# golmschenk/sr-gan

Hardware: AMD Instinct MI355X
Metric: SRGAN train images/sec (G+D step) (higher is better)
Workload: dtype f32; 1 GPU; crowd SRGAN (KnnDenseNetCat D/DNN + DCGenerator) 512x512, batch 16/GPU, dnn_training_step + gan_training_step per step; global_batch=16, image_size=512, schedule=shared-forwards, parallelism=dp1, random_init_weights=True, gradient_penalty=active, launch=eager (Python tape enqueues every kernel), schedule_check=not run: the --full option runs it

## Files before the change

### include/srgan_hip.h

```cpp
#ifndef SRGAN_HIP_H
#define SRGAN_HIP_H

#include <stdint.h>

#ifdef __cplusplus
extern "C" {
#endif

int srgan_version(void);
const char* srgan_build_id(void);
const char* srgan_last_error(void);

#define SRGAN_DTYPE_F32 0x1u
#define SRGAN_DTYPE_BF16 0x2u
#define SRGAN_DTYPE_F16 0x4u
#define SRGAN_FEATURE_FUSED_BNRELU 0x1u
#define SRGAN_FEATURE_SPLITK_WORKSPACE 0x2u
#define SRGAN_FEATURE_LIVE_PROFILE 0x4u
#define SRGAN_FEATURE_BLOCKED16 0x8u
typedef struct srgan_capabilities_t {
  int32_t abi_version;
  int32_t struct_bytes;
  char arch[16];
  uint32_t dtypes;
// ... 46 lines not shown
  float* g_gamma;
  float* g_beta;
} srgan_bn_reduce_job;
int64_t srgan_conv2d_bwd_data_bnrelu_tiles(const srgan_conv_desc* desc);
int srgan_conv2d_bwd_data_bnrelu_partials(const srgan_conv_desc* desc, const float* gy, const float* w, const srgan_bn_relu* bn,
                                          const float* x, float* gx, float* partials, int accumulate, void* stream);
int srgan_bn_partial_reduce_batched(const srgan_bn_reduce_job* jobs_device, int32_t count, int32_t max_channels, int32_t max_tiles,
                                    const float* scratch, void* stream);

int srgan_wgrad_group_plan(const srgan_conv_desc* desc, const srgan_bn_relu* bn, int64_t x_offset, int64_t gy_offset, float* gw,
                           int64_t gw_offset, int32_t group_size, int64_t group_weights, int64_t partial_offset, void* job,
                           int32_t* grid_x, int32_t* grid_y, int32_t* ragged, int64_t* partial_floats);
int srgan_wgrad_group_run(const void* jobs, int32_t count, int32_t kernel_size, int32_t grid_x, int32_t grid_y, int32_t ragged,
                          int32_t fused_bn, const float* x_base, const float* gy_base, float* gw_base, int64_t sum_co_ci_taps,
                          int64_t pixels, int64_t operand_elements, int64_t partial_floats, void* stream);

int srgan_gemm_f32(int32_t M, int32_t N, int32_t K, const float* A, int64_t sai, int64_t sak, const float* B,
                   int64_t sbk, int64_t sbj, float* C, int64_t sci, int64_t scj, const float* bias,
                   int32_t bias_on_columns, int accumulate, int force_kernel, void* stream);
int srgan_gemm(int32_t M, int32_t N, int32_t K, const float* A, int64_t sai, int64_t sak, const float* B,
               int64_t sbk, int64_t sbj, float* C, int64_t sci, int64_t scj, const float* bias,
               int32_t bias_on_columns, int accumulate, int force_kernel, int compute_dtype, void* stream);

int srgan_ew_unary(int op, const float* x, float* y, int64_t n, float p0, float p1, void* stream);
int srgan_ew_binary(int op, const float* a, const float* b, float* y, int64_t n, float p0, void* stream);
int srgan_fill(float* y, int64_t n, float value, void* stream);

int srgan_chan_affine(const float* x, const float* mean, const float* scale_a, const float* scale_b, const float* shift,
                      float* y, int32_t N, int32_t C, int64_t HW, void* stream);

int srgan_chan_affine_act(const float* x, const float* mean, const float* scale_a, const float* scale_b,
                          const float* shift, const float* mask, int relu, float* y, int32_t N, int32_t C, int64_t HW,
                          void* stream);
int srgan_chan_affine_act_strided(const float* x, const float* mean, const float* scale_a, const float* scale_b,
                                  const float* shift, const float* mask, int relu, float* y, int32_t N, int32_t C,
                                  int64_t HW, int64_t x_batch_stride, int64_t mask_batch_stride, int64_t y_batch_stride,
                                  int accumulate, void* stream);
int srgan_bn_conv_tangent_weights(const float* w, const float* q, const float* inv_std, const float* gamma,
                                  float* w_scaled, float* w_grad, float* gamma_grad, int32_t CO, int32_t CI, int32_t taps,
                                  void* stream);

int srgan_bn_conv_tangent_weights_job(const float* w, const float* inv_std, const float* gamma, float* w_grad,
                                      float* gamma_grad, int64_t offset, int32_t CO, int32_t CI, int32_t taps, void* job);
int srgan_bn_conv_tangent_weights_grouped(const void* jobs, int32_t count, int32_t max_inner, int32_t max_co, float* scaled_base,
                                          const float* q_base, void* stream);

int srgan_bn_act_bwd(const float* g, const float* x, const float* mean, const float* inv_std, const float* gamma,
                     const float* beta, int relu, float* gx, float* g_gamma, float* g_beta, int32_t N, int32_t C,
                     int64_t HW, int64_t g_batch_stride, int64_t x_batch_stride, int64_t gx_batch_stride,
                     int accumulate_gx, int unscaled, void* stream);

int srgan_chan_reduce(const float* a, const float* b, const float* mean, const float* scale, float* out, int32_t N,
                      int32_t C, int64_t HW, int accumulate, void* stream);
int srgan_row_max(const float* x, float* out, int32_t B, int32_t F, void* stream);
int srgan_nearest_bin_onehot(const float* y, const float* bins, float* onehot, int32_t B, int32_t K, void* stream);

int srgan_copy_channels(const float* src, int32_t src_channels, int32_t src_first, float* dst, int32_t dst_channels,
                        int32_t dst_first, int32_t count, int32_t N, int64_t HW, int accumulate, void* stream);

int srgan_bn_relu_maxpool_fwd(const float* x, const float* mean, const float* inv_std, const float* gamma, const float* beta,
                              float* y, int32_t* argmax, int32_t N, int32_t C, int32_t H, int32_t W, int32_t k, int32_t s, int32_t p,
                              int32_t OH, int32_t OW, void* stream);
int srgan_bn_relu_maxpool_bwd_supported(int32_t N, int32_t C, int32_t H, int32_t W, int32_t k, int32_t s, int32_t p);
int srgan_bn_relu_maxpool_bwd(const float* gy, const int32_t* argmax, const float* x, const float* mean, const float* inv_std,
                              const float* gamma, const float* beta, float* gx, float* g_gamma, float* g_beta, int32_t N,
                              int32_t C, int32_t H, int32_t W, int32_t k, int32_t s, int32_t p, int32_t OH, int32_t OW,
                              void* stream);
int srgan_bn_relu_avgpool2_supported(int32_t N, int32_t C, int32_t H, int32_t W);
int srgan_bn_relu_avgpool2_fwd(const float* x, const float* mean, const float* inv_std, const float* gamma, const float* beta,
                               float* y, int32_t N, int32_t C, int32_t H, int32_t W, void* stream);
int srgan_bn_relu_avgpool2_bwd(const float* gy, const float* x, const float* mean, const float* inv_std, const float* gamma,
                               const float* beta, float* gx, float* g_gamma, float* g_beta, int32_t N, int32_t C, int32_t H,
                               int32_t W, void* stream);
int srgan_maxpool2d_fwd(const float* x, float* y, int32_t* argmax, int32_t planes, int32_t H, int32_t W, int32_t k,
                        int32_t s, int32_t p, int32_t OH, int32_t OW, void* stream);
int srgan_maxpool2d_bwd(const float* g, const int32_t* argmax, float* gx, int32_t planes, int32_t H, int32_t W, int32_t k,
                        int32_t s, int32_t p, int32_t OH, int32_t OW, void* stream);
int srgan_pool_scatter(const float* g, const int32_t* argmax, float* out, int32_t planes, int64_t in_plane,
                       int64_t out_plane, void* stream);
int srgan_pool_gather(const float* src, const int32_t* argmax, float* out, int32_t planes, int64_t in_plane,
                      int64_t out_plane, void* stream);
int srgan_avgpool2d_fwd(const float* x, float* y, int32_t planes, int32_t H, int32_t W, int32_t k, int32_t s,
                        int32_t OH, int32_t OW, void* stream);
int srgan_avgpool2d_bwd(const float* g, float* gx, int32_t planes, int32_t H, int32_t W, int32_t k, int32_t s,
                        int32_t OH, int32_t OW, void* stream);

int srgan_gp_interpolate(const float* unlabeled, const float* fake, const float* alpha, float* out, int32_t B,
                         int64_t F, void* stream);
int srgan_crowd_map_l1_fwd(const float* maps, const float* target, float* rows, int32_t B, int32_t Cm, int64_t HW,
                           void* stream);
int srgan_crowd_map_l1_bwd(const float* maps, const float* target, const float* g_rows, float* g_maps, int32_t B,
                           int32_t Cm, int64_t HW, void* stream);
int srgan_crowd_extract_patches(const void* const* images_u8, const float* const* labels, const float* const* maps,
                                const int32_t* heights, const int32_t* widths, const int32_t* ys, const int32_t* xs,
                                const int32_t* flips, int32_t B, int32_t P, float* out_images, float* out_labels,
                                float* out_maps, void* stream);

int srgan_crowd_iknn_map(const float* heads_yx, int32_t M, int32_t H, int32_t W, int32_t k, float epsilon, float upper_bound,
                         float* out, void* stream);
int srgan_crowd_density_label(const float* heads, int32_t M, int32_t H, int32_t W, float beta, const float* perspective,
                              int32_t flags, void* workspace, float* out, void* stream);

int srgan_adam_step(float* p, const float* g, float* m, float* v, int64_t n, float lr, float beta1, float beta2,
                    float eps, float weight_decay, int32_t step, void* stream);
int srgan_adam_step_counted(float* p, const float* g, float* m, float* v, int64_t n, float lr, float beta1, float beta2,
                            float eps, float weight_decay, int32_t* state, void* stream);
// ... 62 lines not shown
```

### sr-gan_amd/_lib.py

```python
import ctypes
import os

from ._build import LIBRARY, source_id

c_float_p = ctypes.c_void_p
i32, i64, f32, vp = ctypes.c_int32, ctypes.c_int64, ctypes.c_float, ctypes.c_void_p


class ConvDesc(ctypes.Structure):
    _fields_ = [(name, i32) for name in ('N', 'C', 'H', 'W', 'K', 'R', 'S', 'stride_h', 'stride_w', 'pad_h', 'pad_w',
                                         'OH', 'OW')] + [('x_batch_stride', i64), ('y_batch_stride', i64), ('compute_dtype', i32)]


class BnRelu(ctypes.Structure):
    _fields_ = [(name, vp) for name in ('mean', 'inv_std', 'gamma', 'beta')]


class BnReduceJob(ctypes.Structure):
    _fields_ = [('partial_offset', i64), ('tiles', i32), ('channels', i32), ('inv_std', vp), ('g_gamma', vp), ('g_beta', vp)]


class Capabilities(ctypes.Structure):
    _fields_ = [('abi_version', i32), ('struct_bytes', i32), ('arch', ctypes.c_char * 16), ('dtypes', ctypes.c_uint32),
                ('features', ctypes.c_uint32), ('workspace_bytes', i64), ('max_tensor_elements', i64)]


SIGNATURES = {
    'srgan_version': ([], ctypes.c_int),
    'srgan_build_id': ([], ctypes.c_char_p),
    'srgan_last_error': ([], ctypes.c_char_p),
    'srgan_conv2d_fwd': ([ctypes.POINTER(ConvDesc), vp, vp, vp, vp, ctypes.c_int, vp], ctypes.c_int),
    'srgan_conv2d_bwd_data': ([ctypes.POINTER(ConvDesc), vp, vp, vp, vp, ctypes.c_int, ctypes.c_int, vp],
                              ctypes.c_int),
    'srgan_conv2d_bwd_weight': ([ctypes.POINTER(ConvDesc), vp, vp, vp, ctypes.c_int, ctypes.c_int, vp], ctypes.c_int),
    'srgan_conv2d_bnrelu_supported': ([ctypes.POINTER(ConvDesc), ctypes.c_int], ctypes.c_int),
    'srgan_conv2d_fwd_bnrelu': ([ctypes.POINTER(ConvDesc), vp, ctypes.POINTER(BnRelu), vp, vp, vp, vp], ctypes.c_int),
    'srgan_conv2d_fwd_bnrelu_into_zeros': ([ctypes.POINTER(ConvDesc), vp, ctypes.POINTER(BnRelu), vp, vp, vp, vp],
                                           ctypes.c_int),
    'srgan_conv2d_fwd_bnrelu_splits': ([ctypes.POINTER(ConvDesc)], ctypes.c_int),
    'srgan_bn_conv_tangent_weights': ([vp, vp, vp, vp, vp, vp, vp, i32, i32, i32, vp], ctypes.c_int),
    'srgan_conv2d_bwd_data_bnrelu': ([ctypes.POINTER(ConvDesc), vp, vp, ctypes.POINTER(BnRelu), vp, vp, vp, vp,
                                      ctypes.c_int, vp], ctypes.c_int),
    'srgan_conv2d_bwd_data_bnrelu_tiles': ([ctypes.POINTER(ConvDesc)], ctypes.c_int64),
    'srgan_conv2d_bwd_data_bnrelu_partials': ([ctypes.POINTER(ConvDesc), vp, vp, ctypes.POINTER(BnRelu), vp, vp, vp,
                                               ctypes.c_int, vp], ctypes.c_int),
    'srgan_bn_partial_reduce_batched': ([vp, i32, i32, i32, vp, vp], ctypes.c_int),
    'srgan_conv2d_bwd_weight_bnrelu': ([ctypes.POINTER(ConvDesc), vp, ctypes.POINTER(BnRelu), vp, vp, ctypes.c_int, vp],
                                       ctypes.c_int),
    'srgan_gemm_f32': ([i32, i32, i32, vp, i64, i64, vp, i64, i64, vp, i64, i64, vp, i32, ctypes.c_int, ctypes.c_int,
                        vp], ctypes.c_int),
    'srgan_gemm': ([i32, i32, i32, vp, i64, i64, vp, i64, i64, vp, i64, i64, vp, i32, ctypes.c_int, ctypes.c_int,
                    ctypes.c_int, vp], ctypes.c_int),
    'srgan_ew_unary': ([ctypes.c_int, vp, vp, i64, f32, f32, vp], ctypes.c_int),
    'srgan_ew_binary': ([ctypes.c_int, vp, vp, vp, i64, f32, vp], ctypes.c_int),
    'srgan_fill': ([vp, i64, f32, vp], ctypes.c_int),
    'srgan_chan_affine': ([vp, vp, vp, vp, vp, vp, i32, i32, i64, vp], ctypes.c_int),
    'srgan_chan_affine_act': ([vp, vp, vp, vp, vp, vp, ctypes.c_int, vp, i32, i32, i64, vp], ctypes.c_int),
    'srgan_chan_affine_act_strided': ([vp, vp, vp, vp, vp, vp, ctypes.c_int, vp, i32, i32, i64, i64, i64, i64,
                                       ctypes.c_int, vp], ctypes.c_int),
    'srgan_bn_act_bwd': ([vp, vp, vp, vp, vp, vp, ctypes.c_int, vp, vp, vp, i32, i32, i64, i64, i64, i64, ctypes.c_int,
                          ctypes.c_int, vp],
                         ctypes.c_int),
    'srgan_chan_reduce': ([vp, vp, vp, vp, vp, i32, i32, i64, ctypes.c_int, vp], ctypes.c_int),
    'srgan_row_max': ([vp, vp, i32, i32, vp], ctypes.c_int),
    'srgan_nearest_bin_onehot': ([vp, vp, vp, i32, i32, vp], ctypes.c_int),
    'srgan_copy_channels': ([vp, i32, i32, vp, i32, i32, i32, i32, i64, ctypes.c_int, vp], ctypes.c_int),
    'srgan_bn_relu_maxpool_fwd': ([vp, vp, vp, vp, vp, vp, vp, i32, i32, i32, i32, i32, i32, i32, i32, i32, vp], ctypes.c_int),
    'srgan_bn_relu_maxpool_bwd_supported': ([i32, i32, i32, i32, i32, i32, i32], ctypes.c_int),
    'srgan_bn_relu_maxpool_bwd': ([vp, vp, vp, vp, vp, vp, vp, vp, vp, vp, i32, i32, i32, i32, i32, i32, i32, i32, i32, vp],
                                  ctypes.c_int),
    'srgan_bn_relu_avgpool2_supported': ([i32, i32, i32, i32], ctypes.c_int),
    'srgan_bn_relu_avgpool2_fwd': ([vp, vp, vp, vp, vp, vp, i32, i32, i32, i32, vp], ctypes.c_int),
    'srgan_bn_relu_avgpool2_bwd': ([vp, vp, vp, vp, vp, vp, vp, vp, vp, i32, i32, i32, i32, vp], ctypes.c_int),
    'srgan_maxpool2d_fwd': ([vp, vp, vp, i32, i32, i32, i32, i32, i32, i32, i32, vp], ctypes.c_int),
    'srgan_maxpool2d_bwd': ([vp, vp, vp, i32, i32, i32, i32, i32, i32, i32, i32, vp], ctypes.c_int),
    'srgan_pool_scatter': ([vp, vp, vp, i32, i64, i64, vp], ctypes.c_int),
    'srgan_pool_gather': ([vp, vp, vp, i32, i64, i64, vp], ctypes.c_int),
    'srgan_avgpool2d_fwd': ([vp, vp, i32, i32, i32, i32, i32, i32, i32, vp], ctypes.c_int),
    'srgan_avgpool2d_bwd': ([vp, vp, i32, i32, i32, i32, i32, i32, i32, vp], ctypes.c_int),
    'srgan_gp_interpolate': ([vp, vp, vp, vp, i32, i64, vp], ctypes.c_int),
    'srgan_crowd_map_l1_fwd': ([vp, vp, vp, i32, i32, i64, vp], ctypes.c_int),
    'srgan_crowd_map_l1_bwd': ([vp, vp, vp, vp, i32, i32, i64, vp], ctypes.c_int),
    'srgan_profile_begin': ([], ctypes.c_int),
    'srgan_profile_end': ([ctypes.POINTER(ctypes.c_double), ctypes.POINTER(ctypes.c_double),
                           ctypes.POINTER(ctypes.c_double), ctypes.POINTER(ctypes.c_int64)], ctypes.c_int),
    'srgan_profile_report': ([ctypes.c_char_p, ctypes.c_int64], ctypes.c_int64),
    'srgan_profile_bytes': ([ctypes.POINTER(ctypes.c_double)], ctypes.c_int),
    'srgan_profile_mixed': ([ctypes.POINTER(ctypes.c_double), ctypes.POINTER(ctypes.c_double)], ctypes.c_int),
    'srgan_capabilities': ([ctypes.POINTER(Capabilities), i32], ctypes.c_int),
    'srgan_workspace_bytes': ([], ctypes.c_int64),
    'srgan_set_workspace': ([vp, i64, vp], ctypes.c_int),
    'srgan_split_is_ordered': ([vp], ctypes.c_int),
    'srgan_crowd_density_label': ([vp, i32, i32, i32, f32, vp, i32, vp, vp, vp], ctypes.c_int),
    'srgan_crowd_iknn_map': ([vp, i32, i32, i32, i32, f32, f32, vp, vp], ctypes.c_int),
    'srgan_crowd_extract_patches': ([vp, vp, vp, vp, vp, vp, vp, vp, i32, i32, vp, vp, vp, vp], ctypes.c_int),
    'srgan_bn_conv_tangent_weights_job': ([vp, vp, vp, vp, vp, i64, i32, i32, i32, vp], ctypes.c_int),
    'srgan_bn_conv_tangent_weights_grouped': ([vp, i32, i32, i32, vp, vp, vp], ctypes.c_int),
    'srgan_wgrad_group_plan': ([ctypes.POINTER(ConvDesc), ctypes.POINTER(BnRelu), i64, i64, vp, i64, i32, i64, i64, vp, ctypes.POINTER(i32),
                                ctypes.POINTER(i32), ctypes.POINTER(i32), ctypes.POINTER(i64)], ctypes.c_int),
    'srgan_wgrad_group_run': ([vp, i32, i32, i32, i32, i32, i32, vp, vp, vp, i64, i64, i64, i64, vp], ctypes.c_int),
    'srgan_adam_step': ([vp, vp, vp, vp, i64, f32, f32, f32, f32, f32, i32, vp], ctypes.c_int),
    'srgan_adam_step_counted': ([vp, vp, vp, vp, i64, f32, f32, f32, f32, f32, vp, vp], ctypes.c_int),
    'srgan_pack_bf16': ([vp, vp, i64, vp], ctypes.c_int),
    'srgan_unpack_bf16': ([vp, vp, i64, vp], ctypes.c_int),
    'srgan_h_pack': ([vp, vp, vp, f32, i32, i32, i64, ctypes.c_int, vp], ctypes.c_int),
    'srgan_h_unpack': ([vp, vp, i32, i32, i64, ctypes.c_int, vp], ctypes.c_int),
    'srgan_h_add': ([vp, vp, vp, i64, ctypes.c_int, vp], ctypes.c_int),
    'srgan_h_channel_sums': ([vp, vp, i32, i32, i64, ctypes.c_int, vp], ctypes.c_int),
    'srgan_h_maxpool2': ([vp, vp, vp, i64, i32, i32, ctypes.c_int, ctypes.c_int, vp], ctypes.c_int),
    'srgan_h_maxpool2_bwd': ([vp, vp, vp, i64, i32, i32, ctypes.c_int, f32, ctypes.c_int, vp], ctypes.c_int),
    'srgan_h_conv_weight_slots': ([i32, i32, i32, i32], ctypes.c_int64),
    'srgan_h_pack_conv_weights': ([vp, vp, i32, i32, i32, i32, ctypes.c_int, ctypes.c_int, vp], ctypes.c_int),
    'srgan_h_conv3x3': ([vp, vp, vp, vp, f32, ctypes.c_int, vp, i32, i32, i32, i32, i32, i32, ctypes.c_int, vp], ctypes.c_int),
    'srgan_h_conv3x3_wgrad': ([vp, vp, vp, i32, i32, i32, i32, i32, ctypes.c_int, vp], ctypes.c_int),
    'srgan_h_pack_matrix': ([vp, vp, i64, i64, i64, i64, i64, i64, i32, i32, ctypes.c_int, vp], ctypes.c_int),
# ... 86 lines not shown
```

### sr-gan_amd/crowd/models.py

```python
from collections import OrderedDict

from torch import nn as torch_nn

from .. import functional as F
from .. import nn
from .. import fused
from ..age.models import Generator as _DCGANGenerator, convolution, LEAK
from ..utility import seed_all


FUSED_STEM_POOL = True


class DCGenerator(_DCGANGenerator):

    def __init__(self, z_dim=256, image_size=224, conv_dim=64):
        super().__init__(z_dim=z_dim, image_size=image_size, conv_dim=conv_dim)


class JointDCDiscriminator(nn.Module):

    def __init__(self, image_size=128, conv_dim=64, number_of_outputs=1):
        seed_all(0)
        super().__init__()
        self.number_of_outputs = number_of_outputs
        self.layer1 = convolution(3, conv_dim, 4, bn=False)
        self.layer2 = convolution(conv_dim, conv_dim * 2, 4)
        self.layer3 = convolution(conv_dim * 2, conv_dim * 4, 4)
        self.layer4 = convolution(conv_dim * 4, conv_dim * 8, 4)
        self.count_layer5 = convolution(conv_dim * 8, self.number_of_outputs, int(image_size / 16), 1, 0, False)
        self.density_layer5 = convolution(conv_dim * 8, int(image_size / 4) ** 2, int(image_size / 16), 1, 0, False)
        self.features = None

    def forward(self, x):
        out = x
        for stage in (self.layer1, self.layer2, self.layer3, self.layer4):
            out = F.leaky_relu(stage(out), LEAK)
        self.features = F.flatten2d(out)
        count = self.count_layer5(out)
        count = F.view(count, (-1,) if self.number_of_outputs == 1 else (-1, self.number_of_outputs))
        side = int(x.shape[2] / 4)
        density = F.view(self.density_layer5(out), (-1, side, side))
        return density, count


class _DenseLayer(nn.Sequential):

    def __init__(self, num_input_features, growth_rate, bn_size, drop_rate=0):
        super().__init__()
        self.add_module('norm1', nn.BatchNorm2d(num_input_features))
        self.add_module('relu1', nn.ReLU(inplace=True))
        self.add_module('conv1', nn.Conv2d(num_input_features, bn_size * growth_rate, kernel_size=1, stride=1,
                                           bias=False))
        self.add_module('norm2', nn.BatchNorm2d(bn_size * growth_rate))
        self.add_module('relu2', nn.ReLU(inplace=True))
        self.add_module('conv2', nn.Conv2d(bn_size * growth_rate, growth_rate, kernel_size=3, stride=1, padding=1,
                                           bias=False))
        if drop_rate:
            raise NotImplementedError('drop_rate > 0 is never used on the hot path (crowd/models.py:1063)')
# ... 4 lines not shown


class _DenseBlock(nn.Sequential):
    def __init__(self, num_layers, num_input_features, bn_size, growth_rate, drop_rate=0):
        super().__init__()
        for i in range(num_layers):
            self.add_module('denselayer%d' % (i + 1),
                            _DenseLayer(num_input_features + i * growth_rate, growth_rate, bn_size, drop_rate))

    def forward(self, x):
        if not fused.ENABLED:
            return super().forward(x)
        return fused.dense_block(x, list(self.children()))


class _Transition(nn.Sequential):
    def __init__(self, num_input_features, num_output_features):
        super().__init__()
        self.add_module('norm', nn.BatchNorm2d(num_input_features))
        self.add_module('relu', nn.ReLU(inplace=True))
        self.add_module('conv', nn.Conv2d(num_input_features, num_output_features, kernel_size=1, stride=1,
                                          bias=False))
        self.add_module('pool', nn.AvgPool2d(kernel_size=2, stride=2))

    def forward(self, x):
        if fused.POOL_FIRST:
            pooled = None
            if fused.ENABLED and self.pool.kernel_size == 2 and self.pool.stride == 2:
                inv_std, mean = self.norm._inverse_std()
                pooled = F.bn_relu_avg_pool2d(x, mean, inv_std, nn.P(self.norm.weight), nn.P(self.norm.bias))
            if pooled is None:
                pooled = self.pool(self.norm(x, relu=True))
            return self.conv(pooled)
        y = fused.bn_relu_conv(x, self.norm, self.conv) if fused.ENABLED else None
        if y is None:
            y = self.conv(self.norm(x, relu=True))
        return self.pool(y)


class MapModule(nn.Module):

    def __init__(self, in_features, input_size, label_size, count_outputs=1):
        super().__init__()
        kernel_size = label_size // input_size
        self.map_transposed_conv_layer = nn.ConvTranspose2d(in_channels=in_features, out_channels=1,
                                                            kernel_size=kernel_size, stride=kernel_size)
        self.conv1 = nn.Conv2d(in_channels=1, out_channels=8, kernel_size=2, stride=2)
        self.conv2 = nn.Conv2d(in_channels=8, out_channels=16, kernel_size=2, stride=2)
        self.conv3 = nn.Conv2d(in_channels=16, out_channels=32, kernel_size=2, stride=2)
        self.linear1 = nn.Conv2d(in_channels=32, out_channels=20, kernel_size=label_size // (2 ** 3))
        self.count_layer = nn.Conv2d(in_channels=20, out_channels=count_outputs, kernel_size=1)

    def forward(self, x):
        map_ = F.leaky_relu(self.map_transposed_conv_layer(x))
        out = F.leaky_relu(self.conv1(map_))
        out = F.leaky_relu(self.conv2(out))
        out = F.leaky_relu(self.conv3(out))
        out = F.leaky_relu(self.linear1(out))
        return map_, self.count_layer(out), out


class KnnDenseNetCat(nn.Module):

    COUNT_OUTPUTS = 1

    def __init__(self, growth_rate=32, block_config=(6, 12, 48, 32), num_init_features=64, bn_size=4, drop_rate=0,
                 pretrained=False, label_patch_size=224, image_size=None):
        super().__init__()
        image_size = image_size or label_patch_size
        self.label_patch_size = image_size
        self.dense_blocks = nn.ModuleList()
        self.transition_layers = nn.ModuleList()
        self.conv_layer1 = nn.Sequential(OrderedDict([
            ('conv0', nn.Conv2d(3, num_init_features, kernel_size=7, stride=2, padding=3, bias=False)),
            ('norm0', nn.BatchNorm2d(num_init_features)),
            ('relu0', nn.ReLU(inplace=True)),
            ('pool0', nn.MaxPool2d(kernel_size=3, stride=2, padding=1))]))
        num_features = num_init_features
        widths = []
        for i, num_layers in enumerate(block_config):
            block = _DenseBlock(num_layers=num_layers, num_input_features=num_features, bn_size=bn_size,
                                growth_rate=growth_rate, drop_rate=drop_rate)
            self.dense_blocks.add_module('denseblock%d' % (i + 1), block)
            num_features = num_features + num_layers * growth_rate
            if i != len(block_config) - 1:
                self.transition_layers.add_module('transition%d' % (i + 1),
                                                  _Transition(num_features, num_features // 2))
                num_features = num_features // 2
                widths.append(num_features)
        self.norm5 = nn.BatchNorm2d(num_features)
        for m in self.modules():
            if isinstance(m, torch_nn.Conv2d):
                torch_nn.init.kaiming_normal_(m.weight.data)
            elif isinstance(m, torch_nn.BatchNorm2d):
                m.weight.data.fill_(1)
                m.bias.data.zero_()
            elif isinstance(m, torch_nn.Linear):
                m.bias.data.zero_()
        if pretrained:
            self.load_torchvision_densenet201(pretrained)
        outputs = self.COUNT_OUTPUTS
        self.map_module1 = MapModule(widths[0], image_size // 8, image_size, count_outputs=outputs)
        self.map_module2 = MapModule(widths[1], image_size // 16, image_size, count_outputs=outputs)
        self.map_module3 = MapModule(widths[2], image_size // 32, image_size, count_outputs=outputs)
        self.final_count_feature_layer = nn.Conv2d(in_channels=num_features, out_channels=20, kernel_size=1)
        self.count_layer = nn.Conv2d(in_channels=20, out_channels=outputs, kernel_size=1)
# ... 15 lines not shown
            if match:
                key = match.group(1) + match.group(2)
            key = key.replace('features.denseblock', 'dense_blocks.denseblock')
            key = key.replace('features.transition', 'transition_layers.transition')
            key = key.replace('features.', '') if 'norm5' in key else key.replace('features.', 'conv_layer1.')
            renamed[key] = value
        return renamed

    def load_torchvision_densenet201(self, source=True):
        import os
        if source is True:
            source = os.environ.get(self.TORCHVISION_WEIGHTS_ENV)
            if not source:
                raise RuntimeError('pretrained=True needs the torchvision densenet201 state dict on disk: set '
                                   f'{self.TORCHVISION_WEIGHTS_ENV} to its path (the reference downloads it, '
                                   'crowd/models.py:1110; this build does not touch the network)')
        if isinstance(source, (str, os.PathLike)):
            import torch
            source = torch.load(source, map_location="cpu")
        self.load_state_dict(self.rename_torchvision_keys(source), strict=True)

    def _density(self, batch_size, like):
        cache = self._density_cache
        if cache is None or cache.shape[0] != batch_size or cache.data.device != like.data.device:
            cache = F.full((batch_size, self.label_patch_size, self.label_patch_size), 0.0, like)
            self._density_cache = cache
        return cache

    def forward(self, x):
        count, map_, hidden = self._heads(x)
        batch_size = x.shape[0]
        self.features = F.cat_channels([F.view(t, (batch_size, -1, 1, 1)) for t in hidden])
        return self._density(batch_size, x), F.view(count, (batch_size,)), map_

    def _heads(self, x):
        batch_size = x.shape[0]
        stem = self.conv_layer1
        out, first = None, stem.conv0(x)
        if FUSED_STEM_POOL and isinstance(stem.pool0.kernel_size, int):
            inv_std, mean = stem.norm0._inverse_std()
            out = F.bn_relu_max_pool2d(first, mean, inv_std, nn.parameter_var(stem.norm0.weight),
                                       nn.parameter_var(stem.norm0.bias), stem.pool0.kernel_size, stem.pool0.stride,
                                       stem.pool0.padding)
        if out is None:
            out = stem.pool0(stem.norm0(first, relu=True))
        t1_out = self.transition_layers.transition1(self.dense_blocks.denseblock1(out))
        t2_out = self.transition_layers.transition2(self.dense_blocks.denseblock2(t1_out))
        t3_out = self.transition_layers.transition3(self.dense_blocks.denseblock3(t2_out))
        db4_out = self.dense_blocks.denseblock4(t3_out)
        n5_relu_out = self.norm5(db4_out, relu=True)
        final_pool = F.avg_pool2d(n5_relu_out, kernel_size=self.final_pool_size, stride=1)
        final_count_features = F.leaky_relu(self.final_count_feature_layer(final_pool))
        final_count = self.count_layer(final_count_features)
        map1, count1, h1 = self.map_module1(t1_out)
        map2, count2, h2 = self.map_module2(t2_out)
        map3, count3, h3 = self.map_module3(t3_out)
        count = F.add(F.add(F.add(count1, count2), count3), final_count)
        return count, F.cat_channels([map1, map2, map3]), (h1, h2, h3, final_count_features)


class KnnDenseNetCatDggan(KnnDenseNetCat):
    COUNT_OUTPUTS = 2

    def __init__(self, *args, **kwargs):
        super().__init__(*args, **kwargs)
        self.real_label = None

    def forward(self, x):
        outputs, map_, _ = self._heads(x)
        batch_size = x.shape[0]
        self.real_label = F.view(F.slice_channels(outputs, 1, 2), (batch_size,))
        return self._density(batch_size, x), F.view(F.slice_channels(outputs, 0, 1), (batch_size,)), map_
```

### sr-gan_amd/functional.py

```python
import math
import os

import torch

from . import _lib
from .tape import Var, Node, grad_enabled, no_grad, accumulates_into

U_COPY, U_NEG, U_ABS, U_SIGN, U_SQRT, U_EXP, U_LOG, U_LOG1P, U_SQUARE, U_RECIP, U_TANH, U_RELU, U_STEP, U_AFFINE, \
    U_POW, U_LEAKY, U_SIGMOID, U_SOFTPLUS, U_ONE_MINUS_SQ, U_RSQRT = range(20)
B_ADD, B_SUB, B_MUL, B_DIV, B_DIV_SAFE, B_MAX, B_LEAKY_MASK_MUL, B_AXPY = range(8)

FORCE_KERNEL = 0

COMPUTE_DTYPES = {'f32': 0, 'fp32': 0, 'bf16': 1, 'f16': 2, 'fp16': 2}
COMPUTE_DTYPE = 0


STORAGE_DTYPE = 0
STORAGE_BLOCKED_F32 = 4


class storage_dtype:

    def __init__(self, name):
# ... 173 lines not shown


def sign(x):
    return Var(_unary_raw(U_SIGN, x.data))


def abs_(x):
    return _unary(U_ABS, x, lambda g, needs: (mul(g, sign(x)),), 'abs')


def sqrt(x):
    out = _unary(U_SQRT, x, None, 'sqrt')
    if out.node is not None:
        out.node.backward = lambda g, needs: (div(scale(g, 0.5), out),)
    return out


def exp(x):
    out = _unary(U_EXP, x, None, 'exp')
    if out.node is not None:
        out.node.backward = lambda g, needs: (mul(g, out),)
    return out


def log(x):
    return _unary(U_LOG, x, lambda g, needs: (div(g, x),), 'log')


def log1p(x):
    return _unary(U_LOG1P, x, lambda g, needs: (div(g, add_scalar(x, 1.0)),), 'log1p')


def square(x):
    return _unary(U_SQUARE, x, lambda g, needs: (mul(scale(g, 2.0), x),), 'square')


def one_minus_square(y):
    return _unary(U_ONE_MINUS_SQ, y, lambda g, needs: (scale(mul(g, y), -2.0),), 'one_minus_square')


def tanh(x):
    out = _unary(U_TANH, x, None, 'tanh')
    if out.node is not None:
        out.node.backward = lambda g, needs: (mul(g, one_minus_square(out)),)
    return out


def relu(x):
    return _unary(U_RELU, x, lambda g, needs: (mask_mul(g, x, 0.0),), 'relu')


def leaky_relu(x, negative_slope=0.01):
    return _unary(U_LEAKY, x, lambda g, needs: (mask_mul(g, x, negative_slope),), 'leaky_relu', negative_slope)


def pow_scalar(x, p):
    if p == 2:
        return square(x)
    if p == 1:
        return x
    return _unary(U_POW, x, lambda g, needs: (mul(g, scale(pow_scalar(x, p - 1.0), p)),), 'pow', p)


def sigmoid(x):
    out = _unary(U_SIGMOID, x, None, 'sigmoid')
    if out.node is not None:
        out.node.backward = lambda g, needs: (mul(g, sub(out, square(out))),)
    return out


def softplus(x):
    return _unary(U_SOFTPLUS, x, lambda g, needs: (mul(g, sigmoid(x)),), 'softplus')


def view(x, shape):
    shape = tuple(shape)
    original = x.shape
    return _out(x.data.view(shape), (x,), lambda g, needs: (view(g, original),), 'view')


def flatten2d(x):
    return view(x, (x.shape[0], -1))


def _dims_nchw(shape):
    if len(shape) < 2:
        raise ValueError('need at least [N, C]')
    hw = 1
    for extent in shape[2:]:
        hw *= extent
    return shape[0], shape[1], hw


def chan_affine(x, mean=None, scale_a=None, scale_b=None, shift=None, dims=None, out_shape=None):
    reference = x if x is not None else next(v for v in (scale_a, scale_b, shift) if v is not None)
    if dims is None:
        dims = _dims_nchw(x.shape)
    if out_shape is None:
        out_shape = x.shape
    n, c, hw = dims
    data = _empty(out_shape, reference.data)
    if data.numel() != n * c * hw:
        raise ValueError(f'chan_affine: dims {dims} do not match shape {tuple(out_shape)}')
    for vector in (mean, scale_a, scale_b, shift):
        if vector is not None and vector.numel() != c:
            raise ValueError(f'chan_affine: vector of {vector.numel()} elements for {c} channels')
# ... 101 lines not shown
    return chan_reduce(x, None, dims=(rows, x.numel() // rows, 1))


def row_broadcast(s, shape):
    rows = shape[0]
    count = 1
    for extent in shape[1:]:
        count *= extent
    return chan_affine(None, None, view(s, (rows,)) if s.shape != (rows,) else s, None, None,
                       dims=(1, rows, count), out_shape=tuple(shape))


def col_broadcast(v, rows):
    width = v.numel()
    return chan_affine(None, None, view(v, (width,)) if v.shape != (width,) else v, None, None,
                       dims=(rows, width, 1), out_shape=(rows, width))


def row_norm(x):
    with no_grad():
        out = sqrt(row_dot(x, x))
    if not (grad_enabled() and x.requires_grad):
        return out
    result = Var(out.data, requires_grad=True)
    result.node = Node((x,), lambda g, needs: (row_scale(x, div_safe(g, result)),), 'row_norm')
    return result


def _conv_desc(x_shape, w_shape, stride, padding, y_shape):
    n, c, h, w = x_shape
    k, c2, r, s = w_shape
    if c != c2:
        raise ValueError(f'conv: input has {c} channels, weight expects {c2}')
    return _lib.ConvDesc(n, c, h, w, k, r, s, stride[0], stride[1], padding[0], padding[1], y_shape[2], y_shape[3], 0, 0,
                         COMPUTE_DTYPE)


def _pair(value):
    return (value, value) if isinstance(value, int) else tuple(value)


def conv_output_shape(x_shape, w_shape, stride, padding):
    n, _, h, w = x_shape
    k, _, r, s = w_shape
    return (n, k, (h + 2 * padding[0] - r) // stride[0] + 1, (w + 2 * padding[1] - s) // stride[1] + 1)


def conv2d(x, weight, bias=None, stride=1, padding=0):
    stride, padding = _pair(stride), _pair(padding)
    y_shape = conv_output_shape(x.shape, weight.shape, stride, padding)
    desc = _conv_desc(x.shape, weight.shape, stride, padding, y_shape)
    data = _empty(y_shape, x.data)
    _call('srgan_conv2d_fwd', desc, _ptr(x), _ptr(weight), _ptr(bias), data.data_ptr(), FORCE_KERNEL, _stream())
    x_shape, w_shape = x.shape, weight.shape

    def backward(g, needs):
        gx = conv2d_backward_data(g, weight, x_shape, stride, padding) if needs[0] else None
        gw = gb = None
        if needs[1] and accumulates_into(weight):
            _call('srgan_conv2d_bwd_weight', _conv_desc(x_shape, w_shape, stride, padding, g.shape), _ptr(x), _ptr(g),
                  weight.grad_buffer.data_ptr(), 1, FORCE_KERNEL, _stream())
        elif needs[1]:
            gw = conv2d_backward_weight(x, g, w_shape, stride, padding)
        if needs[2] and accumulates_into(bias):
            _bias_gradient_into(bias.grad_buffer, g)
        elif needs[2]:
            gb = chan_reduce(g)
        return gx, gw, gb
    return _out(data, (x, weight, bias), backward, 'conv2d')


def _bias_gradient_into(buffer, g):
    n, c, hw = _dims_nchw(g.shape)
    _call('srgan_chan_reduce', _ptr(g), None, None, None, buffer.data_ptr(), n, c, hw, 1, _stream())


def conv2d_backward_data(gy, weight, x_shape, stride, padding, bias=None):
    x_shape = tuple(x_shape)
    desc = _conv_desc(x_shape, weight.shape, stride, padding, gy.shape)
    data = _empty(x_shape, gy.data)
    _call('srgan_conv2d_bwd_data', desc, _ptr(gy), _ptr(weight), _ptr(bias), data.data_ptr(), 0, FORCE_KERNEL, _stream())
    w_shape = weight.shape

    def backward(g, needs):
        ggy = conv2d(g, weight, None, stride, padding) if needs[0] else None
        gw = gb = None
        if needs[1] and accumulates_into(weight):
            _call('srgan_conv2d_bwd_weight', _conv_desc(g.shape, w_shape, stride, padding, gy.shape), _ptr(g), _ptr(gy),
                  weight.grad_buffer.data_ptr(), 1, FORCE_KERNEL, _stream())
        elif needs[1]:
            gw = conv2d_backward_weight(g, gy, w_shape, stride, padding)
        if needs[2] and accumulates_into(bias):
            _bias_gradient_into(bias.grad_buffer, g)
        elif needs[2]:
            gb = chan_reduce(g)
        return ggy, gw, gb
    return _out(data, (gy, weight, bias), backward, 'conv2d_backward_data')


def conv2d_backward_weight(x, gy, w_shape, stride, padding):
    w_shape = tuple(w_shape)
    desc = _conv_desc(x.shape, w_shape, stride, padding, gy.shape)
    data = _empty(w_shape, x.data)
    _call('srgan_conv2d_bwd_weight', desc, _ptr(x), _ptr(gy), data.data_ptr(), 0, FORCE_KERNEL, _stream())
    x_shape = x.shape

# ... 294 lines not shown
```

Baseline: 87.68 images/s.

## Fuse the three discriminator map-head forward chains into one grouped HIP kernel

Adds a fused kernel that computes, in a single launch for all three map heads, the leaky ReLU of the transposed-conv output, the three stride-2 2x2 convolutions with leaky ReLU, and the large linear conv as per-block partial sums, followed by a small finish kernel. Each thread walks an 8x8 pixel patch and keeps intermediates in registers and shared memory. The aim is to remove many small eager launches and intermediate round trips through memory. The backward tape is rebuilt from the stored activations. The conv node for the leaky ReLU after a conv is built with the activated data instead of the pre-activation, which relies on the leaky mask sign being the same either way. The path adds register pressure and a serial reduction over blocks.

```diff
diff --git a/include/srgan_hip.h b/include/srgan_hip.h
--- a/include/srgan_hip.h
+++ b/include/srgan_hip.h
@@ -122,6 +122,9 @@
 
 int srgan_chan_reduce(const float* a, const float* b, const float* mean, const float* scale, float* out, int32_t N,
                       int32_t C, int64_t HW, int accumulate, void* stream);
+int64_t srgan_map_head_fwd_workspace(int32_t heads, int32_t B, int32_t S);
+int srgan_map_head_fwd(int32_t heads, const void* const* tensors, float* partial, int32_t B, int32_t S, float slope,
+                       void* stream);
 int srgan_row_max(const float* x, float* out, int32_t B, int32_t F, void* stream);
 int srgan_nearest_bin_onehot(const float* y, const float* bins, float* onehot, int32_t B, int32_t K, void* stream);
 
diff --git a/sr-gan_amd/_lib.py b/sr-gan_amd/_lib.py
--- a/sr-gan_amd/_lib.py
+++ b/sr-gan_amd/_lib.py
@@ -61,6 +61,8 @@
     'srgan_bn_act_bwd': ([vp, vp, vp, vp, vp, vp, ctypes.c_int, vp, vp, vp, i32, i32, i64, i64, i64, i64, ctypes.c_int,
                           ctypes.c_int, vp],
                          ctypes.c_int),
+    'srgan_map_head_fwd_workspace': ([i32, i32, i32], i64),
+    'srgan_map_head_fwd': ([i32, vp, vp, i32, i32, f32, vp], ctypes.c_int),
     'srgan_chan_reduce': ([vp, vp, vp, vp, vp, i32, i32, i64, ctypes.c_int, vp], ctypes.c_int),
     'srgan_row_max': ([vp, vp, i32, i32, vp], ctypes.c_int),
     'srgan_nearest_bin_onehot': ([vp, vp, vp, i32, i32, vp], ctypes.c_int),
diff --git a/sr-gan_amd/crowd/models.py b/sr-gan_amd/crowd/models.py
--- a/sr-gan_amd/crowd/models.py
+++ b/sr-gan_amd/crowd/models.py
@@ -5,6 +5,7 @@
 from .. import functional as F
 from .. import nn
 from .. import fused
+from ..map_head import map_heads
 from ..age.models import Generator as _DCGANGenerator, convolution, LEAK
 from ..utility import seed_all
 
@@ -115,6 +116,9 @@
         self.count_layer = nn.Conv2d(in_channels=20, out_channels=count_outputs, kernel_size=1)
 
     def forward(self, x):
+        return map_heads([self], [x])[0]
+
+    def primitive_forward(self, x):
         map_ = F.leaky_relu(self.map_transposed_conv_layer(x))
         out = F.leaky_relu(self.conv1(map_))
         out = F.leaky_relu(self.conv2(out))
@@ -236,9 +240,8 @@
         final_pool = F.avg_pool2d(n5_relu_out, kernel_size=self.final_pool_size, stride=1)
         final_count_features = F.leaky_relu(self.final_count_feature_layer(final_pool))
         final_count = self.count_layer(final_count_features)
-        map1, count1, h1 = self.map_module1(t1_out)
-        map2, count2, h2 = self.map_module2(t2_out)
-        map3, count3, h3 = self.map_module3(t3_out)
+        (map1, count1, h1), (map2, count2, h2), (map3, count3, h3) = map_heads(
+            [self.map_module1, self.map_module2, self.map_module3], [t1_out, t2_out, t3_out])
         count = F.add(F.add(F.add(count1, count2), count3), final_count)
         return count, F.cat_channels([map1, map2, map3]), (h1, h2, h3, final_count_features)
 
diff --git a/sr-gan_amd/csrc/map_head.hip b/sr-gan_amd/csrc/map_head.hip
--- /dev/null
+++ b/sr-gan_amd/csrc/map_head.hip
@@ -0,0 +1,213 @@
+#include "common.h"
+#include "blocked16.h"
+
+namespace srgan {
+namespace {
+
+constexpr int MH_THREADS = 256;
+constexpr int MH_HIDDEN = 20;
+constexpr int MH_NB = 1;
+constexpr int MH_MAX_HEADS = 3;
+constexpr int W1_AT = 0, B1_AT = 32, W2_AT = 40, B2_AT = 552, W3_AT = 568, B3_AT = 2616, SMALL = 2648;
+
+struct MapHeadPtrs {
+  const float* pre;
+  const float* w1; const float* b1;
+  const float* w2; const float* b2;
+  const float* w3; const float* b3;
+  const float* wl; const float* bl;
+  float* map;
+  float* c1; float* c2; float* c3;
+  float* hidden;
+};
+
+struct MapHeadParams {
+  MapHeadPtrs head[MH_MAX_HEADS];
+  float* partial;
+  int32_t B, S, blocks;
+  float slope;
+};
+
+__device__ __forceinline__ float leaky(float x, float slope) { return x > 0.f ? x : slope * x; }
+
+__global__ __launch_bounds__(MH_THREADS) void map_head_fwd_kernel(MapHeadParams p) {
+  __shared__ float w[SMALL];
+  __shared__ float red[MH_THREADS / 64][MH_NB * MH_HIDDEN];
+  __shared__ float c3s[32][MH_THREADS];
+  const MapHeadPtrs& h = blockIdx.z == 0 ? p.head[0] : blockIdx.z == 1 ? p.head[1] : p.head[2];
+  for (int i = threadIdx.x; i < SMALL; i += MH_THREADS) {
+    float v;
+    if (i < B1_AT) v = h.w1[i - W1_AT];
+    else if (i < W2_AT) v = h.b1[i - B1_AT];
+    else if (i < B2_AT) v = h.w2[i - W2_AT];
+    else if (i < W3_AT) v = h.b2[i - B2_AT];
+    else if (i < B3_AT) v = h.w3[i - W3_AT];
+    else v = h.b3[i - B3_AT];
+    w[i] = v;
+  }
+  __syncthreads();
+
+  const int64_t S = p.S, H1 = S / 2, H2 = S / 4, P = S / 8, plane = P * P;
+  const int pix = blockIdx.x * MH_THREADS + threadIdx.x;
+  const bool valid = pix < plane;
+  const int py = valid ? pix / (int)P : 0, px = valid ? pix % (int)P : 0;
+  const float slope = p.slope;
+  float part[MH_NB][MH_HIDDEN];
+#pragma unroll
+  for (int i = 0; i < MH_NB; ++i)
+#pragma unroll
+    for (int o = 0; o < MH_HIDDEN; ++o) part[i][o] = 0.f;
+
+#pragma unroll
+  for (int i = 0; i < MH_NB; ++i) {
+    const int64_t b = (int64_t)blockIdx.y * MH_NB + i;
+    if (!valid || b >= p.B) continue;
+    float acc3[32];
+#pragma unroll
+    for (int o = 0; o < 32; ++o) acc3[o] = w[B3_AT + o];
+#pragma unroll 1
+    for (int q = 0; q < 4; ++q) {
+      const int qy = q >> 1, qx = q & 1;
+      asm volatile("" ::: "memory");
+      const int64_t block_at = b * S * S + (8 * py + 4 * qy) * S + 8 * px + 4 * qx;
+      float m[4][4];
+#pragma unroll
+      for (int r = 0; r < 4; ++r) {
+        float4 v = *reinterpret_cast<const float4*>(h.pre + block_at + r * S);
+        v.x = leaky(v.x, slope); v.y = leaky(v.y, slope); v.z = leaky(v.z, slope); v.w = leaky(v.w, slope);
+        *reinterpret_cast<float4*>(h.map + block_at + r * S) = v;
+        m[r][0] = v.x; m[r][1] = v.y; m[r][2] = v.z; m[r][3] = v.w;
+      }
+      float acc2[16];
+#pragma unroll
+      for (int o = 0; o < 16; ++o) acc2[o] = w[B2_AT + o];
+#pragma unroll
+      for (int r = 0; r < 4; ++r) {
+        const int ry = r >> 1, rx = r & 1;
+        const int64_t y1 = 4 * py + 2 * qy + ry, x1 = 4 * px + 2 * qx + rx;
+        float c1v[8];
+#pragma unroll
+        for (int o = 0; o < 8; ++o) {
+          float a = w[B1_AT + o];
+          a = fmaf(w[W1_AT + o * 4 + 0], m[2 * ry][2 * rx], a);
+          a = fmaf(w[W1_AT + o * 4 + 1], m[2 * ry][2 * rx + 1], a);
+          a = fmaf(w[W1_AT + o * 4 + 2], m[2 * ry + 1][2 * rx], a);
+          a = fmaf(w[W1_AT + o * 4 + 3], m[2 * ry + 1][2 * rx + 1], a);
+          c1v[o] = leaky(a, slope);
+          h.c1[((b * 8 + o) * H1 + y1) * H1 + x1] = c1v[o];
+        }
+#pragma unroll
+        for (int o = 0; o < 16; ++o)
+#pragma unroll
+          for (int c = 0; c < 8; ++c) acc2[o] = fmaf(w[W2_AT + (o * 8 + c) * 4 + r], c1v[c], acc2[o]);
+      }
+      const int64_t y2 = 2 * py + qy, x2 = 2 * px + qx;
+#pragma unroll
+      for (int c = 0; c < 16; ++c) {
+        const float v = leaky(acc2[c], slope);
+        h.c2[((b * 16 + c) * H2 + y2) * H2 + x2] = v;
+#pragma unroll
+        for (int o = 0; o < 32; ++o) acc3[o] = fmaf(w[W3_AT + (o * 16 + c) * 4 + q], v, acc3[o]);
+      }
+    }
+#pragma unroll
+    for (int c = 0; c < 32; ++c) {
+      const float v = leaky(acc3[c], slope);
+      h.c3[(b * 32 + c) * plane + pix] = v;
+      c3s[c][threadIdx.x] = v;
+    }
+#pragma unroll 2
+    for (int c = 0; c < 32; ++c) {
+      const float v = c3s[c][threadIdx.x];
+      const float* wl = h.wl + (int64_t)c * plane + pix;
+#pragma unroll
+      for (int o = 0; o < MH_HIDDEN; ++o) part[i][o] = fmaf(wl[(int64_t)o * 32 * plane], v, part[i][o]);
+    }
+  }
+
+  const int lane = threadIdx.x & 63, wave = threadIdx.x >> 6;
+#pragma unroll
+  for (int i = 0; i < MH_NB; ++i)
+#pragma unroll
+    for (int o = 0; o < MH_HIDDEN; ++o) {
+      const float v = wave_sum(part[i][o]);
+      if (lane == 0) red[wave][i * MH_HIDDEN + o] = v;
+    }
+  __syncthreads();
+  if (threadIdx.x < MH_NB * MH_HIDDEN) {
+    const int i = threadIdx.x / MH_HIDDEN, o = threadIdx.x % MH_HIDDEN;
+    const int64_t b = (int64_t)blockIdx.y * MH_NB + i;
+    if (b < p.B) {
+      float s = red[0][threadIdx.x];
+#pragma unroll
+      for (int k = 1; k < MH_THREADS / 64; ++k) s += red[k][threadIdx.x];
+      p.partial[(((int64_t)blockIdx.z * p.B + b) * p.blocks + blockIdx.x) * MH_HIDDEN + o] = s;
+    }
+  }
+}
+
+__global__ __launch_bounds__(MH_THREADS) void map_head_finish_kernel(MapHeadParams p) {
+  const int64_t t = (int64_t)blockIdx.x * MH_THREADS + threadIdx.x;
+  if (t >= (int64_t)p.B * MH_HIDDEN) return;
+  const MapHeadPtrs& h = blockIdx.y == 0 ? p.head[0] : blockIdx.y == 1 ? p.head[1] : p.head[2];
+  const int64_t b = t / MH_HIDDEN;
+  const int o = (int)(t % MH_HIDDEN);
+  const float* src = p.partial + ((int64_t)blockIdx.y * p.B + b) * p.blocks * MH_HIDDEN + o;
+  float s = src[0];
+  for (int k = 1; k < p.blocks; ++k) s += src[(int64_t)k * MH_HIDDEN];
+  h.hidden[t] = leaky(s + h.bl[o], p.slope);
+}
+
+}
+
+int64_t map_head_partial_floats(int32_t heads, int32_t B, int32_t S) {
+  const int64_t plane = (int64_t)(S / 8) * (S / 8);
+  return (int64_t)heads * B * ((plane + MH_THREADS - 1) / MH_THREADS) * MH_HIDDEN;
+}
+
+}
+
+using namespace srgan;
+
+extern "C" {
+
+int64_t srgan_map_head_fwd_workspace(int32_t heads, int32_t B, int32_t S) {
+  if (heads < 1 || heads > MH_MAX_HEADS || B < 1 || S < 8) return 0;
+  return map_head_partial_floats(heads, B, S);
+}
+
+int srgan_map_head_fwd(int32_t heads, const void* const* tensors, float* partial, int32_t B, int32_t S, float slope,
+                       void* stream) {
+  SRGAN_REQUIRE(heads >= 1 && heads <= MH_MAX_HEADS && tensors && partial, SRGAN_EINVAL, "srgan_map_head_fwd arguments");
+  SRGAN_REQUIRE(B >= 1 && S >= 8 && S % 8 == 0, SRGAN_EUNSUPPORTED, "srgan_map_head_fwd: the map size is a multiple of 8");
+  const int64_t plane = (int64_t)(S / 8) * (S / 8);
+  SRGAN_REQUIRE((int64_t)B * 32 * plane < ((int64_t)1 << 31) && (int64_t)B * S * S < ((int64_t)1 << 40), SRGAN_ERANGE,
+                "srgan_map_head_fwd size");
+  MapHeadParams p{};
+  for (int k = 0; k < heads; ++k) {
+    const void* const* t = tensors + 14 * k;
+    for (int j = 0; j < 14; ++j) SRGAN_REQUIRE(t[j] != nullptr, SRGAN_EINVAL, "srgan_map_head_fwd: a null tensor");
+    SRGAN_REQUIRE(((uintptr_t)t[0] & 15) == 0 && ((uintptr_t)t[9] & 15) == 0, SRGAN_EINVAL,
+                  "srgan_map_head_fwd: the map tensors are 16-byte aligned");
+    p.head[k] = MapHeadPtrs{(const float*)t[0], (const float*)t[1], (const float*)t[2], (const float*)t[3],
+                            (const float*)t[4], (const float*)t[5], (const float*)t[6], (const float*)t[7],
+                            (const float*)t[8], (float*)t[9], (float*)t[10], (float*)t[11], (float*)t[12], (float*)t[13]};
+  }
+  p.partial = partial;
+  p.B = B;
+  p.S = S;
+  p.blocks = (int)((plane + MH_THREADS - 1) / MH_THREADS);
+  p.slope = slope;
+  hipStream_t s = (hipStream_t)stream;
+  const int slot = profile_bracket_begin(s);
+  hipLaunchKernelGGL(map_head_fwd_kernel, dim3(p.blocks, (B + MH_NB - 1) / MH_NB, heads), dim3(MH_THREADS), 0, s, p);
+  if (const int status = launch_status()) return status;
+  hipLaunchKernelGGL(map_head_finish_kernel, dim3((unsigned)(((int64_t)B * MH_HIDDEN + MH_THREADS - 1) / MH_THREADS), heads),
+                     dim3(MH_THREADS), 0, s, p);
+  if (const int status = launch_status()) return status;
+  const double sq = (double)S * S;
+  const double bytes = 4.0 * heads * ((double)B * sq * (1 + 1 + 2 + 1 + 0.5) + 20.0 * 32 * plane);
+  return profile_bracket_end_bytes(slot, s, 82, (int64_t)heads * B * (int64_t)sq, 1, 16, MH_THREADS, MH_NB, 1, bytes, 0);
+}
+
+}
diff --git a/sr-gan_amd/functional.py b/sr-gan_amd/functional.py
--- a/sr-gan_amd/functional.py
+++ b/sr-gan_amd/functional.py
@@ -249,6 +249,11 @@
 
 def leaky_relu(x, negative_slope=0.01):
     return _unary(U_LEAKY, x, lambda g, needs: (mask_mul(g, x, negative_slope),), 'leaky_relu', negative_slope)
+
+
+def leaky_relu_node(x, data, negative_slope=0.01):
+    reference = Var(data)
+    return _out(data, (x,), lambda g, needs: (mask_mul(g, reference, negative_slope),), 'leaky_relu')
 
 
 def pow_scalar(x, p):
@@ -456,6 +461,11 @@
     desc = _conv_desc(x.shape, weight.shape, stride, padding, y_shape)
     data = _empty(y_shape, x.data)
     _call('srgan_conv2d_fwd', desc, _ptr(x), _ptr(weight), _ptr(bias), data.data_ptr(), FORCE_KERNEL, _stream())
+    return conv2d_node(x, weight, bias, data, stride, padding)
+
+
+def conv2d_node(x, weight, bias, data, stride=1, padding=0):
+    stride, padding = _pair(stride), _pair(padding)
     x_shape, w_shape = x.shape, weight.shape
 
     def backward(g, needs):
diff --git a/sr-gan_amd/map_head.py b/sr-gan_amd/map_head.py
--- /dev/null
+++ b/sr-gan_amd/map_head.py
@@ -0,0 +1,67 @@
+import ctypes
+
+from . import _lib
+from . import functional as F
+from . import fused
+from .nn import parameter_var as P
+
+SLOPE = 0.01
+HIDDEN = 20
+
+
+def _conv_is(conv, out_channels, in_channels, kernel, stride):
+    return (conv.bias is not None and tuple(conv.weight.shape) == (out_channels, in_channels, kernel, kernel) and
+            tuple(conv.stride) == (stride, stride) and tuple(conv.padding) == (0, 0) and
+            tuple(conv.dilation) == (1, 1) and conv.groups == 1)
+
+
+def _supported(module, x):
+    transposed = module.map_transposed_conv_layer
+    if x.meta is not None or len(x.shape) != 4 or not x.data.is_contiguous():
+        return None
+    n, c, h, w = x.shape
+    k = transposed.kernel_size[0]
+    size = h * k
+    if h != w or tuple(transposed.kernel_size) != (k, k) or tuple(transposed.stride) != (k, k) or \
+            tuple(transposed.padding) != (0, 0) or tuple(transposed.output_padding) != (0, 0) or \
+            transposed.bias is None or tuple(transposed.weight.shape) != (c, 1, k, k) or size % 8:
+        return None
+    if not (_conv_is(module.conv1, 8, 1, 2, 2) and _conv_is(module.conv2, 16, 8, 2, 2) and
+            _conv_is(module.conv3, 32, 16, 2, 2) and _conv_is(module.linear1, HIDDEN, 32, size // 8, 1)):
+        return None
+    return n, size
+
+
+def map_heads(modules, inputs):
+    shapes = [_supported(m, x) for m, x in zip(modules, inputs)] if fused.ENABLED else [None]
+    if any(s is None for s in shapes) or len(set(shapes)) != 1 or len(modules) > 3:
+        return [m.primitive_forward(x) for m, x in zip(modules, inputs)]
+    batch, size = shapes[0]
+    pres = [m.map_transposed_conv_layer(x) for m, x in zip(modules, inputs)]
+    like = pres[0].data
+    pointers, outputs = [], []
+    for module, pre in zip(modules, pres):
+        if pre.meta is not None:
+            return [m.primitive_forward(x) for m, x in zip(modules, inputs)]
+        tensors = (like.new_empty((batch, 1, size, size)), like.new_empty((batch, 8, size // 2, size // 2)),
+                   like.new_empty((batch, 16, size // 4, size // 4)), like.new_empty((batch, 32, size // 8, size // 8)),
+                   like.new_empty((batch, HIDDEN, 1, 1)))
+        outputs.append(tensors)
+        pointers += [pre.data.data_ptr()] + [P(p).data.data_ptr() for p in (
+            module.conv1.weight, module.conv1.bias, module.conv2.weight, module.conv2.bias, module.conv3.weight,
+            module.conv3.bias, module.linear1.weight, module.linear1.bias)] + [t.data_ptr() for t in tensors]
+    library = _lib.library()
+    partial = like.new_empty((max(int(library.srgan_map_head_fwd_workspace(len(modules), batch, size)), 1),))
+    table = (ctypes.c_void_p * len(pointers))(*pointers)
+    _lib.check(library.srgan_map_head_fwd(len(modules), table, partial.data_ptr(), batch, size, SLOPE, F._stream()),
+               'srgan_map_head_fwd')
+    results = []
+    for module, pre, (map_, c1, c2, c3, hidden) in zip(modules, pres, outputs):
+        map_var = F.leaky_relu_node(pre, map_, SLOPE)
+        out = map_var
+        for conv, data in ((module.conv1, c1), (module.conv2, c2), (module.conv3, c3)):
+            out = F.leaky_relu_node(F.conv2d_node(out, P(conv.weight), P(conv.bias), data, 2, 0), data, SLOPE)
+        hidden_var = F.leaky_relu_node(F.conv2d_node(out, P(module.linear1.weight), P(module.linear1.bias), hidden),
+                                       hidden, SLOPE)
+        results.append((map_var, module.count_layer(hidden_var), hidden_var))
+    return results
```

After: 88.12 images/s (median of 6 runs). About the same (+0.5%).
